# Gumo-A/hnsw_rs

Measured on AMD Instinct MI355X. Metric: queries/sec at recall@10>=0.99, 1M x 100d L2, higher is better.
Workload: dtype f32

## Files before the change

### hnsw_rs_amd/csrc/search_lean.hip

```cpp

#include <algorithm>
#include <cstdlib>

#include "device_index.h"
#include "launch.h"
#include "search_common.h"
#include "switches.h"

namespace hx {
namespace {

#define HX_LIKELY(x) __builtin_expect(!!(x), 1)
#define HX_UNLIKELY(x) __builtin_expect(!!(x), 0)

constexpr u64 LK_INVALID = ~0ull;
constexpr u64 LK_MASK = 0x7FFFFFFFFFFFFFFFull;
constexpr u64 LK_EXPANDED = 1ull << 63;

struct LeanArgs {
    const float *rows;
    const uint32_t *adj0;
    const uint32_t *adj_up;
    const uint32_t *upper_base;
    const uint32_t *ovf_off, *ovf_nbrs;
    const float *Q;
    const uint32_t *qsel;
    uint32_t *out_ids;
    float *out_dists;
    uint32_t *out_counts;
    hnsw_query_stats *out_stats;
    uint32_t n_points, ep, nb_layers, S0, S1, ef, n, slots_log2;
    unsigned long long *dbg;
    uint32_t *spill_tab;
    uint32_t spill_log2;
    uint32_t lds_limit;
};

#ifdef HX_STAMPS
__device__ __forceinline__ unsigned long long stamp_now() {
    __builtin_amdgcn_sched_barrier(0);
    asm volatile("s_waitcnt vmcnt(0) lgkmcnt(0)" ::: "memory");
    const unsigned long long t = __builtin_readcyclecounter();
    asm volatile("s_waitcnt lgkmcnt(0)" ::: "memory");
    __builtin_amdgcn_sched_barrier(0);
    return t;
}
#define STAMP(var) const unsigned long long var = stamp_now()
#define STAMP_ADD(slot, a, b) dbg_acc[slot] += (b) - (a)
#else
#define STAMP(var)
#define STAMP_ADD(slot, a, b)
#endif

__device__ __forceinline__ uint32_t rdlane(uint32_t v, uint32_t l) {
    return (uint32_t)__builtin_amdgcn_readlane((int)v, (int)l);
}
__device__ __forceinline__ u64 rdlane64(u64 v, uint32_t l) {
    return ((u64)rdlane((uint32_t)(v >> 32), l) << 32) | rdlane((uint32_t)v, l);
}
__device__ __forceinline__ uint32_t uni(uint32_t x) { return (uint32_t)__builtin_amdgcn_readfirstlane((int)x); }
__device__ __forceinline__ void lds_fence() { asm volatile("s_waitcnt lgkmcnt(0)" ::: "memory"); }
template <int CTRL>
__device__ __forceinline__ uint32_t dpp_or_max(uint32_t x) {
    return (uint32_t)__builtin_amdgcn_update_dpp(-1, (int)x, CTRL, 0xF, 0xF, false);
}
__device__ __forceinline__ uint32_t wave_min_u32(uint32_t v) {
    v = min(v, dpp_or_max<0xB1>(v));
    v = min(v, dpp_or_max<0x4E>(v));
    v = min(v, dpp_or_max<0x141>(v));
    v = min(v, dpp_or_max<0x140>(v));
    return min(min(rdlane(v, 0), rdlane(v, 16)), min(rdlane(v, 32), rdlane(v, 48)));
}

struct Visited {
    uint32_t *tab;
    uint32_t bshift, bmask;

    __device__ __forceinline__ uint32_t home(uint32_t id) const { return (id * 0x9E3779B1u) >> bshift; }

    __device__ __forceinline__ uint32_t look(uint32_t id, uint32_t b) const {
        const uint4 bk = *reinterpret_cast<const uint4 *>(tab + 4 * b);
        const uint32_t m = min(min(bk.x ^ id, bk.y ^ id), min(bk.z ^ id, bk.w ^ id));
        const uint32_t nf = 4u + (uint32_t)(((int32_t)bk.x >> 31) + ((int32_t)bk.y >> 31) + ((int32_t)bk.z >> 31) +
                                            ((int32_t)bk.w >> 31));
        return m == 0 ? 4u : (nf == 4u ? 5u : nf);
    }
    __device__ __forceinline__ uint32_t claim(uint32_t id, uint32_t b, uint32_t t) const {
        uint32_t old = 0;
        if (t < 4u) old = atomicCAS(tab + 4 * b + t, HX_EMPTY_SLOT, id);
        return old;
    }
    __device__ __forceinline__ bool finish(uint32_t id, uint32_t b, uint32_t t, bool pend, bool fresh) const {
        while (__ballot(pend)) {
            if (pend) {
                if (t == 5u) b = (b + 1) & bmask;
                t = look(id, b);
                const uint32_t old = claim(id, b, t);
                const bool won = old == HX_EMPTY_SLOT;
                fresh |= won;
                pend = (t != 4u) & !won;
            }
        }
        return fresh;
    }
    __device__ __forceinline__ bool insert(uint32_t id, bool ins) const {
        const uint32_t b = home(id);
        uint32_t t = look(id, b);
        t = ins ? t : 4u;
        const uint32_t old = claim(id, b, t);
        const bool fresh = old == HX_EMPTY_SLOT;
        return finish(id, b, t, (t != 4u) & !fresh, fresh);
    }
    __device__ __forceinline__ void clear(uint32_t nslots, int lane) const {
        for (uint32_t s = lane; s < (nslots >> 2); s += 64)
            reinterpret_cast<uint4 *>(tab)[s] = make_uint4(HX_EMPTY_SLOT, HX_EMPTY_SLOT, HX_EMPTY_SLOT, HX_EMPTY_SLOT);
        lds_fence();
    }

    uint32_t *gtab = nullptr;
    uint32_t gshift = 0, gmask = 0;
    bool spill = false;

    __device__ __forceinline__ bool g_contains(uint32_t id) const {
        uint32_t s = ((id * 0x9E3779B1u) >> gshift) & gmask;
        while (true) {
            const uint32_t cur = __hip_atomic_load(gtab + s, __ATOMIC_RELAXED, __HIP_MEMORY_SCOPE_AGENT);
            if (cur == id) return true;
            if (cur == HX_EMPTY_SLOT) return false;
            s = (s + 1) & gmask;
        }
    }
    __device__ __forceinline__ uint32_t g_claim(uint32_t id) const {
        uint32_t s = ((id * 0x9E3779B1u) >> gshift) & gmask;
        while (true) {
            const uint32_t old = atomicCAS(gtab + s, HX_EMPTY_SLOT, id);
            if (old == HX_EMPTY_SLOT) return HX_EMPTY_SLOT;
            if (old == id) return id;
            s = (s + 1) & gmask;
        }
    }
    __device__ __forceinline__ void open_second_level(int lane) {
        const uint32_t nslots = gmask + 1;
        for (uint32_t s = lane; s < (nslots >> 2); s += 64)
            reinterpret_cast<uint4 *>(gtab)[s] = make_uint4(HX_EMPTY_SLOT, HX_EMPTY_SLOT, HX_EMPTY_SLOT, HX_EMPTY_SLOT);
        __builtin_amdgcn_fence(__ATOMIC_RELEASE, "agent");
        asm volatile("s_waitcnt vmcnt(0)" ::: "memory");
        spill = true;
    }
    __device__ __forceinline__ uint32_t look2(uint32_t id, uint32_t b, bool probe, bool claim_now) const {
        uint32_t t = look(id, b);
        if (!spill) return t;
        if (!probe) return 4u;
        while (t == 5u) {
            b = (b + 1) & bmask;
            t = look(id, b);
        }
        if (t == 4u) return 4u;
        if (claim_now) return g_claim(id) == HX_EMPTY_SLOT ? 7u : 4u;
        return g_contains(id) ? 4u : 6u;
    }
    __device__ __forceinline__ uint32_t claim2(uint32_t id, uint32_t b, uint32_t t) const {
        uint32_t old = 0;
        if (t < 4u)
            old = atomicCAS(tab + 4 * b + t, HX_EMPTY_SLOT, id);
        else if (t == 6u)
            old = g_claim(id);
        else if (t == 7u)
            old = HX_EMPTY_SLOT;
        return old;
    }
    __device__ __forceinline__ bool finish2(uint32_t id, uint32_t b, uint32_t t, bool pend, bool fresh) const {
        while (__ballot(pend)) {
            if (pend) {
                if (t == 5u) b = (b + 1) & bmask;
                t = look2(id, b, true, false);
                const uint32_t old = claim2(id, b, t);
                const bool won = old == HX_EMPTY_SLOT;
                fresh |= won;
                pend = (t != 4u) & !won;
            }
        }
        return fresh;
    }
};

#ifndef HX_MERGE_SHIFT_MAX
#define HX_MERGE_SHIFT_MAX 2
#endif
template <int R>
struct Lst {
    static constexpr int NR = R;
    struct Masks {
        u64 U[R];
    };
    u64 L[R];
    uint32_t n_cur;
    u64 last_key;

    static __device__ __forceinline__ uint32_t idx_of(int r, int lane) { return (uint32_t)(R * lane + r); }
    __device__ __forceinline__ void set_first(u64 key, int lane) {
        if (lane == 0) L[0] = key;
        n_cur = 1;
    }

    __device__ __forceinline__ void init() {
#pragma unroll
        for (int r = 0; r < R; r++) L[r] = LK_INVALID;
        n_cur = 0;
        last_key = LK_INVALID;
    }
    __device__ __forceinline__ int first_unexp() const {
        uint32_t pos = 0xFFFFFFFFu;
#pragma unroll
        for (int r = 0; r < R; r++) {
            const u64 U = __ballot((int32_t)(uint32_t)(L[r] >> 32) >= 0);
            const uint32_t i = U ? (uint32_t)(R * (__ffsll((long long)U) - 1) + r) : 0xFFFFFFFFu;
            pos = min(pos, i);
        }
        return (int)pos;
    }
    __device__ __forceinline__ void unexp_masks(Masks &mk) const {
#pragma unroll
        for (int r = 0; r < R; r++) mk.U[r] = __ballot((int32_t)(uint32_t)(L[r] >> 32) >= 0);
    }
    __device__ __forceinline__ int take_first(Masks &mk) const {
        u64(&U)[R] = mk.U;
        uint32_t pos = 0xFFFFFFFFu;
#pragma unroll
        for (int r = 0; r < R; r++) {
            const uint32_t i = U[r] ? (uint32_t)(R * (__ffsll((long long)U[r]) - 1) + r) : 0xFFFFFFFFu;
            pos = min(pos, i);
        }
#pragma unroll
        for (int r = 0; r < R; r++)
            if (pos != 0xFFFFFFFFu && (pos % R) == (uint32_t)r) U[r] &= U[r] - 1;
        return (int)pos;
    }
    __device__ __forceinline__ uint32_t id_at(uint32_t pos) const {
        uint32_t v = 0;
#pragma unroll
        for (int r = 0; r < R; r++) {
            const uint32_t t = rdlane((uint32_t)L[r], pos / R);
            if ((pos % R) == (uint32_t)r) v = t;
        }
        return v;
    }
    __device__ __forceinline__ u64 key_at(uint32_t pos) const {
        u64 v = 0;
#pragma unroll
        for (int r = 0; r < R; r++) {
            const u64 t = rdlane64(L[r], pos / R);
            if ((pos % R) == (uint32_t)r) v = t;
        }
        return v;
    }
    __device__ __forceinline__ void mark(uint32_t pos, int lane) {
#pragma unroll
        for (int r = 0; r < R; r++)
            if ((pos % R) == (uint32_t)r && (uint32_t)lane == pos / R) L[r] |= LK_EXPANDED;
    }
    __device__ __forceinline__ void refresh_last(uint32_t ef) {
        last_key = n_cur >= ef ? (key_at(ef - 1) & LK_MASK) : LK_INVALID;
    }

    __device__ __forceinline__ void merge(u64 key, uint32_t ef, u64 *perm, int lane) {
        const bool surv = key < last_key;
        const u64 smask = __ballot(surv);
        if (smask == 0) return;
        const uint32_t m = (uint32_t)__popcll(smask);
        if (m <= HX_MERGE_SHIFT_MAX) {
            u64 it = smask;
            while (it) {
                const uint32_t j = (uint32_t)__ffsll((long long)it) - 1;
                it &= it - 1;
                const u64 e = rdlane64(key, j);
                if (!(e < last_key)) continue;
                uint32_t pos = 0;
#pragma unroll
                for (int r = 0; r < R; r++) pos += (uint32_t)__popcll(__ballot((L[r] & LK_MASK) < e));
                const uint32_t plo = (uint32_t)__builtin_amdgcn_update_dpp(0, (int)(uint32_t)L[R - 1], 0x138, 0xF, 0xF, false);
                const uint32_t phi = (uint32_t)__builtin_amdgcn_update_dpp(0, (int)(uint32_t)(L[R - 1] >> 32), 0x138, 0xF, 0xF, false);
                u64 below = ((u64)phi << 32) | plo;
#pragma unroll
                for (int r = R - 1; r >= 0; r--) {
                    const uint32_t idx = (uint32_t)(R * lane + r);
                    const u64 from = r > 0 ? L[r > 0 ? r - 1 : 0] : below;
                    L[r] = idx < pos ? L[r] : (idx == pos ? e : from);
                }
                n_cur = min(n_cur + 1, ef);
                if (ef < 64u * R) {
#pragma unroll
                    for (int r = 0; r < R; r++)
                        if ((uint32_t)(R * lane + r) >= ef) L[r] = LK_INVALID;
                }
                refresh_last(ef);
            }
            return;
        }
        u64 *sv = perm + 64 * R;
        u64 Lm[R];
        uint32_t shift[R];
#pragma unroll
        for (int r = 0; r < R; r++) {
            Lm[r] = L[r] & LK_MASK;
            shift[r] = 0;
        }
        uint32_t srank = 0;
        u64 it = smask;
        while (it) {
            const uint32_t j = (uint32_t)__ffsll((long long)it) - 1;
            it &= it - 1;
            const u64 e = rdlane64(key, j);
#pragma unroll
            for (int r = 0; r < R; r++) shift[r] += e < Lm[r] ? 1u : 0u;
            srank += e < key ? 1u : 0u;
        }
        const uint32_t n_new = min(n_cur + m, ef);
#pragma unroll
        for (int r = 0; r < R; r++) perm[R * lane + r] = LK_INVALID;
        asm volatile("" ::: "memory");
#pragma unroll
        for (int r = 0; r < R; r++) {
            const uint32_t idx = (uint32_t)(R * lane + r);
            const uint32_t np = idx + shift[r];
            if (idx < n_cur && np < n_new) perm[np] = L[r];
        }
        if (surv) sv[srank] = key;
        asm volatile("" ::: "memory");
        u64 v[R], H[R];
        bool hole[R];
#pragma unroll
        for (int r = 0; r < R; r++) v[r] = perm[R * lane + r];
#pragma unroll
        for (int r = 0; r < R; r++) {
            hole[r] = v[r] == LK_INVALID && (uint32_t)(R * lane + r) < n_new;
            H[r] = __ballot(hole[r]);
        }
#pragma unroll
        for (int r = 0; r < R; r++) {
            uint32_t hr = 0;
#pragma unroll
            for (int r2 = 0; r2 < R; r2++) {
                hr += __builtin_amdgcn_mbcnt_hi((uint32_t)(H[r2] >> 32), __builtin_amdgcn_mbcnt_lo((uint32_t)H[r2], 0u));
                if (r2 < r && hole[r2]) hr++;
            }
            if (hole[r]) v[r] = sv[hr];
        }
#pragma unroll
        for (int r = 0; r < R; r++) L[r] = v[r];
        n_cur = n_new;
        lds_fence();
        refresh_last(ef);
    }
};

struct LstHT {
    static constexpr int NR = 2;
    struct Masks {
        u64 head, tail;
        bool tail_known;
    };
    u64 L[2];
    uint32_t n_cur;
    u64 last_key;

    static __device__ __forceinline__ uint32_t idx_of(int r, int lane) { return (uint32_t)(64 * r + lane); }
    __device__ __forceinline__ void init() {
        L[0] = L[1] = LK_INVALID;
        n_cur = 0;
        last_key = LK_INVALID;
    }
    __device__ __forceinline__ void set_first(u64 key, int lane) {
        if (lane == 0) L[0] = key;
        n_cur = 1;
    }
    __device__ __forceinline__ void unexp_masks(Masks &mk) const {
        mk.head = __ballot((int32_t)(uint32_t)(L[0] >> 32) >= 0);
        mk.tail = 0;
        mk.tail_known = false;
    }
    __device__ __forceinline__ int take_first(Masks &mk) const {
        if (HX_LIKELY(mk.head != 0)) {
            const int pos = __ffsll((long long)mk.head) - 1;
            mk.head &= mk.head - 1;
            return pos;
        }
        if (!mk.tail_known) {
            mk.tail = n_cur > 64 ? __ballot((int32_t)(uint32_t)(L[1] >> 32) >= 0) : 0ull;
            mk.tail_known = true;
        }
        if (mk.tail == 0) return -1;
        const int pos = __ffsll((long long)mk.tail) - 1;
        mk.tail &= mk.tail - 1;
        return 64 + pos;
    }
    __device__ __forceinline__ uint32_t id_at(uint32_t pos) const {
        const uint32_t a = rdlane((uint32_t)L[0], pos & 63u), b = rdlane((uint32_t)L[1], pos & 63u);
        return pos < 64u ? a : b;
    }
    __device__ __forceinline__ u64 key_at(uint32_t pos) const {
        const u64 a = rdlane64(L[0], pos & 63u), b = rdlane64(L[1], pos & 63u);
        return pos < 64u ? a : b;
    }
    __device__ __forceinline__ void mark(uint32_t pos, int lane) {
        if ((uint32_t)lane == pos) L[0] |= LK_EXPANDED;
        if ((uint32_t)lane + 64u == pos) L[1] |= LK_EXPANDED;
    }
    __device__ __forceinline__ void refresh_last(uint32_t ef) {
        last_key = n_cur >= ef ? (rdlane64(L[1], (ef - 65u) & 63u) & LK_MASK) : LK_INVALID;
    }
    static __device__ __forceinline__ u64 shr1(u64 v) {
        const uint32_t lo = (uint32_t)__builtin_amdgcn_update_dpp(0, (int)(uint32_t)v, 0x138, 0xF, 0xF, false);
        const uint32_t hi = (uint32_t)__builtin_amdgcn_update_dpp(0, (int)(uint32_t)(v >> 32), 0x138, 0xF, 0xF, false);
        return ((u64)hi << 32) | lo;
    }

    __device__ __forceinline__ void merge(u64 key, uint32_t ef, u64 *perm, int lane) {
        const bool surv = key < last_key;
        const u64 smask = __ballot(surv);
        if (smask == 0) return;
        const uint32_t m = (uint32_t)__popcll(smask);
        if (m <= HX_MERGE_SHIFT_MAX) {
            u64 it = smask;
            while (it) {
                const uint32_t j = (uint32_t)__ffsll((long long)it) - 1;
                it &= it - 1;
                const u64 e = rdlane64(key, j);
                if (!(e < last_key)) continue;
                const uint32_t pos = (uint32_t)__popcll(__ballot((L[0] & LK_MASK) < e));
                if (pos < 64u) {
                    const u64 carry = rdlane64(L[0], 63);
                    const u64 below = shr1(L[0]);
                    L[0] = (uint32_t)lane < pos ? L[0] : ((uint32_t)lane == pos ? e : below);
                    const u64 tb = shr1(L[1]);
                    L[1] = lane == 0 ? carry : tb;
                } else {
                    const uint32_t tpos = (uint32_t)__popcll(__ballot((L[1] & LK_MASK) < e));
                    const u64 tb = shr1(L[1]);
                    L[1] = (uint32_t)lane < tpos ? L[1] : ((uint32_t)lane == tpos ? e : tb);
                }
                n_cur = min(n_cur + 1, ef);
                if (64u + (uint32_t)lane >= ef) L[1] = LK_INVALID;
                refresh_last(ef);
            }
            return;
        }
        u64 *sv = perm + 128;
        const u64 Mm = L[0] & LK_MASK, Tm = L[1] & LK_MASK;
        uint32_t sh0 = 0, sh1 = 0, srank = 0;
        u64 it = smask;
        while (it) {
            const uint32_t j = (uint32_t)__ffsll((long long)it) - 1;
            it &= it - 1;
            const u64 e = rdlane64(key, j);
            sh0 += e < Mm ? 1u : 0u;
            sh1 += e < Tm ? 1u : 0u;
            srank += e < key ? 1u : 0u;
        }
        const uint32_t n_new = min(n_cur + m, ef);
        perm[lane] = LK_INVALID;
        perm[64 + lane] = LK_INVALID;
        asm volatile("" ::: "memory");
        {
            const uint32_t i0 = (uint32_t)lane, i1 = 64u + (uint32_t)lane;
            if (i0 < n_cur && i0 + sh0 < n_new) perm[i0 + sh0] = L[0];
            if (i1 < n_cur && i1 + sh1 < n_new) perm[i1 + sh1] = L[1];
        }
        if (surv) sv[srank] = key;
        asm volatile("" ::: "memory");
        u64 v0 = perm[lane], v1 = perm[64 + lane];
        const bool hole0 = v0 == LK_INVALID && (uint32_t)lane < n_new;
        const bool hole1 = v1 == LK_INVALID && 64u + (uint32_t)lane < n_new;
        const u64 H0 = __ballot(hole0), H1 = __ballot(hole1);
        const uint32_t hr0 = __builtin_amdgcn_mbcnt_hi((uint32_t)(H0 >> 32), __builtin_amdgcn_mbcnt_lo((uint32_t)H0, 0u));
        const uint32_t hr1 = (uint32_t)__popcll(H0) +
                             __builtin_amdgcn_mbcnt_hi((uint32_t)(H1 >> 32), __builtin_amdgcn_mbcnt_lo((uint32_t)H1, 0u));
        if (hole0) v0 = sv[hr0];
        if (hole1) v1 = sv[hr1];
        L[0] = v0;
        L[1] = v1;
        n_cur = n_new;
        lds_fence();
        refresh_last(ef);
    }
};

template <int DS>
__device__ __forceinline__ float chain_sum(const uint4 (&w)[DS / 4], const float (&qv)[DS]) {
    float s = 0.0f;
#pragma unroll
    for (int p = 0; p < DS / 4; p++) {
        const uint32_t dw[4] = {w[p].x, w[p].y, w[p].z, w[p].w};
#pragma unroll
        for (int j = 0; j < 4; j += 2) {
            const f32x2 x = {__builtin_bit_cast(float, dw[j]), __builtin_bit_cast(float, dw[j + 1])};
            const f32x2 y = {qv[4 * p + j], qv[4 * p + j + 1]};
            const f32x2 t = x - y;
            const f32x2 t2 = t * t;
            s += t2.x;
            s += t2.y;
        }
    }
    return s;
}
template <int DS>
__device__ __forceinline__ float row_dist(const float *rows, uint32_t id, bool want, const float (&qv)[DS]) {
    float s = 0.0f;
    if (want) {
        const uint4 *src = reinterpret_cast<const uint4 *>(rows + (size_t)id * DS);
        uint4 w[DS / 4];
#pragma unroll
        for (int p = 0; p < DS / 4; p++) w[p] = src[p];
        __builtin_amdgcn_sched_barrier(0);
        s = chain_sum<DS>(w, qv);
    }
    return __builtin_sqrtf(s);
}

template <int DS, class LT, int CK = 4>
__global__ void __launch_bounds__(64) hx_lean_f32_kernel(const LeanArgs a) {
    constexpr int R = LT::NR;
    static_assert(DS % 4 == 0, "whole 16-byte pieces");
    constexpr bool COOP = coop_rows<HNSW_VEC_F32, DS>();
    constexpr bool SPILLV = R >= 6;
    extern __shared__ __attribute__((aligned(16))) unsigned char smem[];
    const int lane = threadIdx.x;
    const uint32_t q = a.qsel ? a.qsel[blockIdx.x] : blockIdx.x;
    const uint32_t hslots = 1u << a.slots_log2;
    u64 *perm = reinterpret_cast<u64 *>(smem + 4ull * hslots);
    unsigned char *coop_img = reinterpret_cast<unsigned char *>(perm);
    uint32_t *coop_ids = reinterpret_cast<uint32_t *>(coop_img + HX_COOP_IMG_BYTES);
    Visited vis;
    vis.tab = reinterpret_cast<uint32_t *>(smem);

    uint32_t n_dist = 0, n_exp = 0, sum_deg = 0, n_vis = 0;
    int32_t status = HNSW_OK;
#ifdef HX_STAMPS
    unsigned long long dbg_acc[16] = {0, 0, 0, 0, 0, 0, 0, 0, 0, 0, 0, 0, 0, 0, 0, 0};
    const unsigned long long t_begin = __builtin_readcyclecounter();
#endif

    const float *qp = a.Q + (size_t)q * DS;
    QueryRegs<DS> qreg;
    float(&qv)[DS] = qreg.v;
#pragma unroll
    for (int e = 0; e < DS; e++) qv[e] = qp[e];
    {
        bool bad = false;
        for (int e = lane; e < DS; e += 64) {
            const float x = qp[e];
            bad |= (x != x);
        }
        if (__ballot(bad)) status = HNSW_ERR_NAN_INPUT;
    }
#pragma unroll
    for (int e = 0; e < DS; e++) asm volatile("" : "+v"(qv[e]));

    auto dist_of = [&](uint32_t id, bool want) __attribute__((always_inline)) -> float {
        if constexpr (COOP) {
            return __builtin_sqrtf(f32_rows_coop<DS, CK, true, true>(reinterpret_cast<const uint8_t *>(a.rows), id, want, qreg,
                                                                    coop_ids, coop_img, lane));
        } else {
            return row_dist<DS>(a.rows, id, want, qv);
        }
    };

    u64 best = LK_INVALID;
    uint32_t cur = a.ep;
    if (status == HNSW_OK) {
        if (cur >= a.n_points) {
            status = HNSW_ERR_ARG;
        } else {
            const float d0 = dist_of(cur, lane == 0);
            const uint32_t bits = rdlane(__builtin_bit_cast(uint32_t, d0), 0);
            n_dist = 1;
            if (__builtin_bit_cast(float, bits) != __builtin_bit_cast(float, bits))
                status = HNSW_ERR_NAN_INPUT;
            else
                best = ((u64)bits << 32) | cur;
        }
    }

    const uint32_t up_slots = max(hslots >> 2, 64u);
    uint32_t ub_cur = HX_EMPTY_SLOT;
    bool have_ub = false;
    for (int layer = (int)a.nb_layers - 1; layer >= 1 && status == HNSW_OK; layer--) {
        vis.bshift = 32 - (__ffs((int)up_slots) - 1 - 2);
        vis.bmask = (up_slots >> 2) - 1;
        const uint32_t vis_limit = up_slots - (up_slots >> 2);
        vis.clear(up_slots, lane);
        vis.insert(cur, lane == 0);
        n_vis = 1;
        if (!have_ub) {
            ub_cur = uni(a.upper_base[cur]);
            have_ub = true;
        }
        while (status == HNSW_OK) {
            if (ub_cur == HX_EMPTY_SLOT) {
                status = HNSW_ERR_NODE_NOT_IN_GRAPH;
                break;
            }
            n_exp++;
            bool improved = false;
            uint32_t new_cur = cur, new_ub = ub_cur;
            const uint32_t *row = a.adj_up + ((size_t)ub_cur + (uint32_t)layer - 1) * a.S1;
            uint32_t ovf_lo = 0, ovf_hi = 0;
            bool first = true;
            while (true) {
                uint32_t nb = HX_EMPTY_SLOT;
                if (first) {
                    if ((uint32_t)lane < a.S1) nb = row[lane];
                } else {
                    if (ovf_lo + lane < ovf_hi) nb = a.ovf_nbrs[ovf_lo + lane];
                    ovf_lo += 64;
                }
                const bool valid = (int32_t)nb >= 0;
                if (first) {
                    const u64 pm = __ballot((int32_t)nb < 0 && nb != HX_EMPTY_SLOT);
                    if (HX_UNLIKELY(pm != 0)) {
                        const uint32_t o = rdlane(nb, (uint32_t)__ffsll((long long)pm) - 1) & ~HX_OVF_FLAG;
                        ovf_lo = uni(a.ovf_off[o]);
                        ovf_hi = uni(a.ovf_off[o + 1]);
                    }
                    first = false;
                }
                const uint32_t cnt = (uint32_t)__popcll(__ballot(valid));
                sum_deg += cnt;
                if (HX_LIKELY(cnt != 0)) {
                    if (HX_UNLIKELY(n_vis + cnt > vis_limit)) {
                        status = HNSW_ERR_OVERFLOW;
                        break;
                    }
                    const bool fresh = vis.insert(nb, valid);
                    const u64 fm = __ballot(fresh);
                    const uint32_t nf = (uint32_t)__popcll(fm);
                    n_vis += nf;
                    n_dist += nf;
                    if (HX_LIKELY(fm != 0)) {
                        uint32_t ubn = HX_EMPTY_SLOT;
                        if (fresh) ubn = a.upper_base[nb];
                        const float dist = dist_of(nb, fresh);
                        const bool nan = fresh && dist != dist;
                        if (HX_UNLIKELY(__ballot(nan) != 0)) {
                            status = HNSW_ERR_NAN_INPUT;
                            break;
                        }
                        const uint32_t db = fresh ? __builtin_bit_cast(uint32_t, dist) : 0xFFFFFFFFu;
                        const uint32_t mn = wave_min_u32(db);
                        u64 tie = __ballot(fresh && db == mn);
                        uint32_t j = (uint32_t)__ffsll((long long)tie) - 1;
                        uint32_t bid = rdlane(nb, j);
                        tie &= tie - 1;
                        while (tie) {
                            const uint32_t j2 = (uint32_t)__ffsll((long long)tie) - 1;
                            tie &= tie - 1;
                            const uint32_t id2 = rdlane(nb, j2);
                            if (id2 < bid) {
                                bid = id2;
                                j = j2;
                            }
                        }
                        const u64 k = ((u64)mn << 32) | bid;
                        if (k < best) {
                            best = k;
                            new_cur = bid;
                            new_ub = rdlane(ubn, j);
                            improved = true;
                        }
                    }
                }
                if (HX_LIKELY(ovf_lo >= ovf_hi)) break;
            }
            if (!improved || status != HNSW_OK) break;
            cur = new_cur;
            ub_cur = new_ub;
        }
    }

#ifdef HX_STAMPS
    dbg_acc[7] = __builtin_readcyclecounter() - t_begin;
#endif
    const uint32_t ef = max(1u, a.ef);
    LT lst;
    lst.init();
    if (status == HNSW_OK) {
        vis.bshift = 32 - (a.slots_log2 - 2);
        vis.bmask = (hslots >> 2) - 1;
        uint32_t lds_limit = hslots - (hslots >> 2);
        if constexpr (SPILLV) {
            if (a.spill_tab != nullptr && a.lds_limit != 0) lds_limit = min(lds_limit, max(128u, a.lds_limit));
        }
        uint32_t vis_limit = lds_limit;
        if constexpr (SPILLV) {
            if (a.spill_tab != nullptr) {
                vis.gtab = a.spill_tab + ((size_t)blockIdx.x << a.spill_log2);
                vis.gmask = (1u << a.spill_log2) - 1;
                vis.gshift = 32 - a.spill_log2;
                vis_limit = lds_limit + (1u << a.spill_log2) / 2;
            }
        }
        vis.clear(hslots, lane);
        vis.insert(cur, lane == 0);
        n_vis = 1;
        lst.set_first(best, lane);
        lst.refresh_last(ef);
        const uint32_t S0 = a.S0;
        const bool upper = lane >= 32;
        const uint32_t slot = (uint32_t)lane & 31u;
        uint32_t pre_nb = HX_EMPTY_SLOT, pre_c = HX_EMPTY_SLOT, pre_p = HX_EMPTY_SLOT;

        uint32_t ovf_lo = 0, ovf_hi = 0;

        while (true) {
            STAMP(f0);
            if constexpr (SPILLV) {
                if (HX_UNLIKELY(!vis.spill && vis.gtab != nullptr && n_vis + 64u > lds_limit)) vis.open_second_level(lane);
            }
            int ppos = -1;
            uint32_t pid = HX_EMPTY_SLOT;
            uint32_t nb = HX_EMPTY_SLOT;
            const bool ovf_pass = ovf_lo < ovf_hi;
            if (HX_UNLIKELY(ovf_pass)) {
                if (lane < 32 && ovf_lo + (uint32_t)lane < ovf_hi) nb = a.ovf_nbrs[ovf_lo + (uint32_t)lane];
                ovf_lo += 32;
            } else {
                typename LT::Masks U;
                lst.unexp_masks(U);
                const int cpos = lst.take_first(U);
                if (HX_UNLIKELY(cpos < 0)) break;
                ppos = lst.take_first(U);
                const uint32_t cid = lst.id_at((uint32_t)cpos);
                if (ppos >= 0) pid = lst.id_at((uint32_t)ppos);
                lst.mark((uint32_t)cpos, lane);
                n_exp++;
                if (HX_LIKELY(pre_c == cid && pre_p == pid)) {
                    nb = pre_nb;
                } else {
                    if (slot < S0 && (!upper || ppos >= 0)) nb = a.adj0[(size_t)(upper ? pid : cid) * S0 + slot];
                }
                pre_c = HX_EMPTY_SLOT;
            }
#ifdef HX_STAMPS
            asm volatile("s_waitcnt vmcnt(0)" ::: "memory");
            dbg_acc[6]++;
#endif
            STAMP(f1);
            STAMP_ADD(0, f0, f1);
            const u64 pm = ovf_pass ? 0ull : __ballot((int32_t)nb < -1);
            const bool spec_ok = ppos >= 0 && (pm >> 32) == 0;
            const bool valid = (int32_t)nb >= 0 && (!upper || spec_ok);
            const uint32_t vb = vis.home(nb);
            uint32_t vt0;
            if constexpr (SPILLV)
                vt0 = vis.look2(nb, vb, valid, valid && !upper);
            else
                vt0 = vis.look(nb, vb);
            const uint32_t vt = valid ? vt0 : 4u;
            const bool want_pre = vt != 4u;
            const uint32_t ct = upper ? 4u : vt;
            bool fresh = false;
            float dist = 0.0f;
            if constexpr (COOP) {
                const uint32_t old = SPILLV ? vis.claim2(nb, vb, ct) : vis.claim(nb, vb, ct);
                fresh = old == HX_EMPTY_SLOT;
                const bool pend = (ct != 4u) & !fresh;
                if (HX_UNLIKELY(__ballot(pend) != 0)) fresh = SPILLV ? vis.finish2(nb, vb, ct, pend, fresh) : vis.finish(nb, vb, ct, pend, fresh);
                dist = dist_of(nb, upper ? want_pre : fresh);
            } else if (want_pre) {
                const uint4 *src = reinterpret_cast<const uint4 *>(a.rows + (size_t)nb * DS);
                uint4 w[DS / 4];
#pragma unroll
                for (int p = 0; p < DS / 4; p++) w[p] = src[p];
                __builtin_amdgcn_sched_barrier(0);
                const uint32_t old = SPILLV ? vis.claim2(nb, vb, ct) : vis.claim(nb, vb, ct);
                fresh = old == HX_EMPTY_SLOT;
                const bool pend = (ct != 4u) & !fresh;
                if (HX_UNLIKELY(__ballot(pend) != 0)) {
                    fresh = SPILLV ? vis.finish2(nb, vb, ct, pend, fresh) : vis.finish(nb, vb, ct, pend, fresh);
#ifdef HX_STAMPS
                    dbg_acc[11]++;
#endif
                }
                __builtin_amdgcn_sched_barrier(0);
#ifdef HX_STAMPS
                __builtin_amdgcn_sched_barrier(0);
                asm volatile("s_waitcnt lgkmcnt(0)" ::: "memory");
                const unsigned long long g0 = __builtin_readcyclecounter();
                asm volatile("s_waitcnt lgkmcnt(0)" ::: "memory");
                const unsigned long long g1 = stamp_now();
                dbg_acc[2] += g1 - g0;
#endif
                const float s = chain_sum<DS>(w, qv);
                dist = __builtin_sqrtf(s);
#ifdef HX_STAMPS
                asm volatile("" ::"v"(dist) : "memory");
                dbg_acc[3] += stamp_now() - g1;
#endif
            }
            const bool want = upper ? want_pre : fresh;
            const u64 vmask = __ballot(valid), fmask = __ballot(fresh);
            const uint32_t cnt_c = (uint32_t)__popcll(vmask & 0xFFFFFFFFull);
            const uint32_t cnt_p = (uint32_t)__popcll(vmask >> 32);
            const uint32_t nf_c = (uint32_t)__popcll(fmask);
            sum_deg += cnt_c;
            n_vis += nf_c;
            n_dist += nf_c;
            if (HX_UNLIKELY(n_vis > vis_limit)) {
                status = HNSW_ERR_OVERFLOW;
                break;
            }
            const bool nan = want && dist != dist;
            u64 key = LK_INVALID;
            if (want && !nan) key = ((u64)__builtin_bit_cast(uint32_t, dist) << 32) | nb;
            STAMP(f2);
            STAMP_ADD(1, f1, f2);
            STAMP(f3);
#ifdef HX_STAMPS
            {
                const uint32_t mm = (uint32_t)__popcll(__ballot(!upper && key < lst.last_key));
                if (mm == 0) dbg_acc[12]++; else if (mm <= 2) dbg_acc[13]++; else dbg_acc[14]++;
            }
#endif
            const u64 nanm = __ballot(nan);
            if (HX_UNLIKELY((nanm & 0xFFFFFFFFull) != 0)) {
                status = HNSW_ERR_NAN_INPUT;
                break;
            }
            lst.merge(upper ? LK_INVALID : key, ef, perm, lane);
            STAMP(f3b);
            STAMP_ADD(8, f3, f3b);
            if (HX_UNLIKELY((pm & 0xFFFFFFFFull) != 0)) {
                const uint32_t c_ovf = rdlane(nb, (uint32_t)__ffsll((long long)(pm & 0xFFFFFFFFull)) - 1) & ~HX_OVF_FLAG;
                ovf_lo = uni(a.ovf_off[c_ovf]);
                ovf_hi = uni(a.ovf_off[c_ovf + 1]);
                if (ovf_lo < ovf_hi) continue;
            }
            if (HX_UNLIKELY(!spec_ok)) continue;
            typename LT::Masks V;
            lst.unexp_masks(V);
            const int npos = lst.take_first(V);
            if (HX_UNLIKELY(npos < 0)) break;
            if (HX_UNLIKELY(lst.id_at((uint32_t)npos) != pid)) continue;
            {
                const int apos = lst.take_first(V);
                if (HX_LIKELY(apos >= 0)) {
                    const int bpos = lst.take_first(V);
                    pre_c = lst.id_at((uint32_t)apos);
                    pre_p = bpos >= 0 ? lst.id_at((uint32_t)bpos) : HX_EMPTY_SLOT;
                    pre_nb = HX_EMPTY_SLOT;
                    if (slot < S0 && (!upper || bpos >= 0)) pre_nb = a.adj0[(size_t)(upper ? pre_p : pre_c) * S0 + slot];
                }
            }
            STAMP(f4);
            STAMP_ADD(9, f3b, f4);
            lst.mark((uint32_t)npos, lane);
            n_exp++;
            const uint32_t pt = upper ? vt : 4u;
            const uint32_t pold = SPILLV ? vis.claim2(nb, vb, pt) : vis.claim(nb, vb, pt);
            bool pfresh = pold == HX_EMPTY_SLOT;
            const bool ppend = (pt == 5u) | ((pt < 4u) & !pfresh & (pold != nb));
            if (HX_UNLIKELY(__ballot(ppend) != 0))
                pfresh = SPILLV ? vis.finish2(nb, vb, pt == 5u ? 5u : 0u, ppend, pfresh) : vis.finish(nb, vb, pt == 5u ? 5u : 0u, ppend, pfresh);
            const uint32_t nf_p = (uint32_t)__popcll(__ballot(pfresh));
            sum_deg += cnt_p;
            n_vis += nf_p;
            n_dist += nf_p;
            if (HX_UNLIKELY(n_vis > vis_limit)) {
                status = HNSW_ERR_OVERFLOW;
                break;
            }
            if (HX_UNLIKELY(__ballot(pfresh && nan) != 0)) {
                status = HNSW_ERR_NAN_INPUT;
                break;
            }
            STAMP(f4b);
            STAMP_ADD(5, f4, f4b);
#ifdef HX_STAMPS
            {
                const uint32_t mm = (uint32_t)__popcll(__ballot(pfresh && key < lst.last_key));
                if (mm == 0) dbg_acc[12]++; else if (mm <= 2) dbg_acc[13]++; else dbg_acc[14]++;
                dbg_acc[15]++;
            }
#endif
            lst.merge(pfresh ? key : LK_INVALID, ef, perm, lane);
            STAMP(f5);
            STAMP_ADD(10, f4b, f5);
        }
    }

    const uint32_t count = status == HNSW_OK ? min(a.n, lst.n_cur) : 0;
#pragma unroll
    for (int r = 0; r < R; r++) {
        const uint32_t idx = LT::idx_of(r, lane);
        if (idx < a.n) {
            const bool have = idx < count;
            a.out_ids[(size_t)q * a.n + idx] = have ? (uint32_t)lst.L[r] : HX_EMPTY_SLOT;
            if (a.out_dists)
                a.out_dists[(size_t)q * a.n + idx] =
                    have ? __builtin_bit_cast(float, (uint32_t)((lst.L[r] & LK_MASK) >> 32)) : __builtin_inff();
        }
    }
    for (uint32_t idx = 64u * R + lane; idx < a.n; idx += 64) {
        a.out_ids[(size_t)q * a.n + idx] = HX_EMPTY_SLOT;
        if (a.out_dists) a.out_dists[(size_t)q * a.n + idx] = __builtin_inff();
    }
#ifdef HX_STAMPS
    if (lane == 0 && a.dbg) {
        dbg_acc[4] = __builtin_readcyclecounter() - t_begin;
        for (int i = 0; i < 16; i++) a.dbg[(size_t)q * 16 + i] = dbg_acc[i];
    }
#endif
    if (lane == 0) {
        if (a.out_counts) a.out_counts[q] = count;
        hnsw_query_stats st;
        st.n_dist = n_dist;
        st.n_exp = n_exp;
        st.sum_deg = sum_deg;
        st.status = status;
        a.out_stats[q] = st;
    }
}

template <class LT>
__global__ void __launch_bounds__(64) hx_lean_q8_kernel(const LeanArgs a) {
    constexpr int R = LT::NR;
    constexpr bool SPILLV = R >= 6;
    constexpr int DS = 100, P = 4, NQ = 4 * (DS / 8) + DS % 8;
    constexpr uint32_t HALF = 64, ROW = 128, NCH4 = 4 * (DS / 8), REM = DS % 8;
    extern __shared__ __attribute__((aligned(16))) unsigned char smem[];
    const int lane = threadIdx.x;
    const int h = lane & 1;
    const uint32_t cslot = (uint32_t)lane >> 1;
    const uint32_t q = a.qsel ? a.qsel[blockIdx.x] : blockIdx.x;
    const uint32_t hslots = 1u << a.slots_log2;
    u64 *perm = reinterpret_cast<u64 *>(smem + 4ull * hslots);
    float *yq = reinterpret_cast<float *>(perm + 64 * R + 64);
    Visited vis;
    vis.tab = reinterpret_cast<uint32_t *>(smem);
    const uint8_t *rows8 = reinterpret_cast<const uint8_t *>(a.rows);

    uint32_t n_dist = 0, n_exp = 0, sum_deg = 0, n_vis = 0;
    int32_t status = HNSW_OK;
#ifdef HX_STAMPS
    unsigned long long dbg_acc[16] = {0, 0, 0, 0, 0, 0, 0, 0, 0, 0, 0, 0, 0, 0, 0, 0};
    const unsigned long long t_begin = __builtin_readcyclecounter();
#endif

    QRegs<NQ> qreg;
    {
        DevView dv{};
        dv.dim = DS;
        dv.half_bytes = HALF;
        dv.nch4 = NCH4;
        dv.rem = REM;
        if (!stage_query<HNSW_VEC_QUANT8>(dv, a.Q + (size_t)q * DS, yq, lane)) status = HNSW_ERR_NAN_INPUT;
#pragma unroll
        for (int e = 0; e < NQ; e++) qreg.v[e] = yq[h * (HALF - 8) + e];
    }
    auto eval = [&](uint32_t id, bool want) __attribute__((always_inline)) -> float {
        float acc[4] = {0.0f, 0.0f, 0.0f, 0.0f};
        if (want) {
            const uint4 *src = reinterpret_cast<const uint4 *>(rows8 + (size_t)id * ROW + (size_t)h * HALF);
            uint4 w[P];
#pragma unroll
            for (int p = 0; p < P; p++) w[p] = src[p];
            __builtin_amdgcn_sched_barrier(0);
            quant_half_sums<P, DS>(w, qreg, h, NCH4, REM, acc);
        }
        const float b0 = pair_swap(acc[0]), b1 = pair_swap(acc[1]), b2 = pair_swap(acc[2]), b3 = pair_swap(acc[3]);
        float s = 0.0f;
        s += acc[0];
        s += acc[1];
        s += acc[2];
        s += acc[3];
        s += b0;
        s += b1;
        s += b2;
        s += b3;
        return __builtin_sqrtf(s);
    };
    auto pair_insert = [&](uint32_t id, bool ins) __attribute__((always_inline)) -> bool {
        bool f;
        if constexpr (SPILLV) {
            const bool mine = ins && h == 0;
            const uint32_t b0 = vis.home(id);
            const uint32_t t0 = vis.look2(id, b0, mine, mine);
            const uint32_t t = mine ? t0 : 4u;
            const uint32_t old = vis.claim2(id, b0, t);
            f = old == HX_EMPTY_SLOT;
            f = vis.finish2(id, b0, t, (t != 4u) & !f, f);
        } else {
            f = vis.insert(id, ins && h == 0);
        }
        return (pair_swap_i(f ? 1 : 0) | (f ? 1 : 0)) != 0;
    };

    u64 best = LK_INVALID;
    uint32_t cur = a.ep;
    if (status == HNSW_OK) {
        if (cur >= a.n_points) {
            status = HNSW_ERR_ARG;
        } else {
            const float d0 = eval(cur, lane < 2);
            const uint32_t bits = rdlane(__builtin_bit_cast(uint32_t, d0), 0);
            n_dist = 1;
            if (__builtin_bit_cast(float, bits) != __builtin_bit_cast(float, bits))
                status = HNSW_ERR_NAN_INPUT;
            else
                best = ((u64)bits << 32) | cur;
        }
    }

    const uint32_t up_slots = max(hslots >> 2, 64u);
    uint32_t ub_cur = HX_EMPTY_SLOT;
    bool have_ub = false;
    for (int layer = (int)a.nb_layers - 1; layer >= 1 && status == HNSW_OK; layer--) {
        vis.bshift = 32 - (__ffs((int)up_slots) - 1 - 2);
        vis.bmask = (up_slots >> 2) - 1;
        const uint32_t vis_limit = up_slots - (up_slots >> 2);
        vis.clear(up_slots, lane);
        vis.insert(cur, lane == 0);
        n_vis = 1;
        if (!have_ub) {
            ub_cur = uni(a.upper_base[cur]);
            have_ub = true;
        }
        while (status == HNSW_OK) {
            if (ub_cur == HX_EMPTY_SLOT) {
                status = HNSW_ERR_NODE_NOT_IN_GRAPH;
                break;
            }
            n_exp++;
            bool improved = false;
            uint32_t new_cur = cur, new_ub = ub_cur;
            const uint32_t *row = a.adj_up + ((size_t)ub_cur + (uint32_t)layer - 1) * a.S1;
            uint32_t ovf_lo = 0, ovf_hi = 0;
            for (uint32_t c0 = 0; c0 < a.S1 || ovf_lo < ovf_hi; c0 += 32) {
                uint32_t nb = HX_EMPTY_SLOT;
                if (c0 < a.S1) {
                    if (c0 + cslot < a.S1) nb = row[c0 + cslot];
                    const u64 pm = __ballot((int32_t)nb < -1);
                    if (HX_UNLIKELY(pm != 0)) {
                        const uint32_t o = rdlane(nb, (uint32_t)__ffsll((long long)pm) - 1) & ~HX_OVF_FLAG;
                        ovf_lo = uni(a.ovf_off[o]);
                        ovf_hi = uni(a.ovf_off[o + 1]);
                    }
                } else {
                    if (ovf_lo + cslot < ovf_hi) nb = a.ovf_nbrs[ovf_lo + cslot];
                    ovf_lo += 32;
                }
                const bool valid = (int32_t)nb >= 0;
                const uint32_t cnt = (uint32_t)__popcll(__ballot(valid && h == 0));
                sum_deg += cnt;
                if (cnt == 0) continue;
                if (n_vis + cnt > vis_limit) {
                    status = HNSW_ERR_OVERFLOW;
                    break;
                }
                const bool fresh = pair_insert(nb, valid);
                const u64 fm = __ballot(fresh && h == 0);
                const uint32_t nf = (uint32_t)__popcll(fm);
                n_vis += nf;
                n_dist += nf;
                if (fm == 0) continue;
                uint32_t ubn = HX_EMPTY_SLOT;
                if (fresh && h == 0) ubn = a.upper_base[nb];
                const float dist = eval(nb, fresh);
                const bool mine = fresh && h == 0;
                if (__ballot(mine && dist != dist)) {
                    status = HNSW_ERR_NAN_INPUT;
                    break;
                }
                const uint32_t db = mine ? __builtin_bit_cast(uint32_t, dist) : 0xFFFFFFFFu;
                const uint32_t mn = wave_min_u32(db);
                u64 tie = __ballot(mine && db == mn);
                uint32_t j = (uint32_t)__ffsll((long long)tie) - 1;
                uint32_t bid = rdlane(nb, j);
                tie &= tie - 1;
                while (tie) {
                    const uint32_t j2 = (uint32_t)__ffsll((long long)tie) - 1;
                    tie &= tie - 1;
                    const uint32_t id2 = rdlane(nb, j2);
                    if (id2 < bid) {
                        bid = id2;
                        j = j2;
                    }
                }
                const u64 k = ((u64)mn << 32) | bid;
                if (k < best) {
                    best = k;
                    new_cur = bid;
                    new_ub = rdlane(ubn, j);
                    improved = true;
                }
            }
            if (!improved || status != HNSW_OK) break;
            cur = new_cur;
            ub_cur = new_ub;
        }
    }

#ifdef HX_STAMPS
    dbg_acc[7] = __builtin_readcyclecounter() - t_begin;
#endif
    const uint32_t ef = max(1u, a.ef);
    LT lst;
    lst.init();
    if (status == HNSW_OK) {
        vis.bshift = 32 - (a.slots_log2 - 2);
        vis.bmask = (hslots >> 2) - 1;
        uint32_t lds_limit = hslots - (hslots >> 2);
        if constexpr (SPILLV) {
            if (a.spill_tab != nullptr && a.lds_limit != 0) lds_limit = min(lds_limit, max(128u, a.lds_limit));
        }
        uint32_t vis_limit = lds_limit;
        if constexpr (SPILLV) {
            if (a.spill_tab != nullptr) {
                vis.gtab = a.spill_tab + ((size_t)blockIdx.x << a.spill_log2);
                vis.gmask = (1u << a.spill_log2) - 1;
                vis.gshift = 32 - a.spill_log2;
                vis_limit = lds_limit + (1u << a.spill_log2) / 2;
            }
        }
        vis.clear(hslots, lane);
        vis.insert(cur, lane == 0);
        n_vis = 1;
        lst.set_first(best, lane);
        lst.refresh_last(ef);
        const uint32_t S0 = a.S0;
        uint32_t pre_nb = HX_EMPTY_SLOT, pre_c = HX_EMPTY_SLOT;

        while (true) {
            STAMP(f0);
            if constexpr (SPILLV) {
                if (HX_UNLIKELY(!vis.spill && vis.gtab != nullptr && n_vis + 64u > lds_limit)) vis.open_second_level(lane);
            }
            typename LT::Masks U;
            lst.unexp_masks(U);
            const int cpos = lst.take_first(U);
            if (cpos < 0) break;
            const int ppos = lst.take_first(U);
            const uint32_t cid = lst.id_at((uint32_t)cpos);
            lst.mark((uint32_t)cpos, lane);
            n_exp++;
            uint32_t nb;
            if (pre_c == cid) {
                nb = pre_nb;
            } else {
                nb = HX_EMPTY_SLOT;
                if (cslot < S0) nb = a.adj0[(size_t)cid * S0 + cslot];
            }
            pre_c = HX_EMPTY_SLOT;
            if (ppos >= 0) {
                pre_c = lst.id_at((uint32_t)ppos);
                pre_nb = HX_EMPTY_SLOT;
                if (cslot < S0) pre_nb = a.adj0[(size_t)pre_c * S0 + cslot];
            }
            const u64 pm = __ballot((int32_t)nb < -1);
#ifdef HX_STAMPS
            dbg_acc[6]++;
#endif
            STAMP(f1);
            STAMP_ADD(0, f0, f1);
            const bool valid = (int32_t)nb >= 0;
            const uint32_t vb = vis.home(nb);
            uint32_t vt0;
            if constexpr (SPILLV)
                vt0 = vis.look2(nb, vb, valid && h == 0, valid && h == 0);
            else
                vt0 = vis.look(nb, vb);
            const uint32_t ct = (valid && h == 0) ? vt0 : 4u;
            const uint32_t old = SPILLV ? vis.claim2(nb, vb, ct) : vis.claim(nb, vb, ct);
            bool fresh0 = old == HX_EMPTY_SLOT;
            const bool pend = (ct != 4u) & !fresh0;
            if (__ballot(pend)) fresh0 = SPILLV ? vis.finish2(nb, vb, ct, pend, fresh0) : vis.finish(nb, vb, ct, pend, fresh0);
            const bool fresh = (pair_swap_i(fresh0 ? 1 : 0) | (fresh0 ? 1 : 0)) != 0;
            const u64 vmask = __ballot(valid && h == 0), fmask = __ballot(fresh0);
            const uint32_t nf = (uint32_t)__popcll(fmask);
            sum_deg += (uint32_t)__popcll(vmask);
            n_vis += nf;
            n_dist += nf;
            if (HX_UNLIKELY(n_vis > vis_limit)) {
                status = HNSW_ERR_OVERFLOW;
                break;
            }
            STAMP(f2);
            STAMP_ADD(1, f1, f2);
            u64 key = LK_INVALID;
            if (fmask) {
                const float dist = eval(nb, fresh);
                const bool mine = fresh0;
                if (__ballot(mine && dist != dist)) {
                    status = HNSW_ERR_NAN_INPUT;
                    break;
                }
                if (mine) key = ((u64)__builtin_bit_cast(uint32_t, dist) << 32) | nb;
            }
            STAMP(f3);
            STAMP_ADD(3, f2, f3);
            lst.merge(key, ef, perm, lane);
            STAMP(f4);
            STAMP_ADD(8, f3, f4);
            if (pm) {
                const uint32_t c_ovf = rdlane(nb, (uint32_t)__ffsll((long long)pm) - 1) & ~HX_OVF_FLAG;
                const uint32_t lo = uni(a.ovf_off[c_ovf]), hi = uni(a.ovf_off[c_ovf + 1]);
                for (uint32_t base = lo; base < hi && status == HNSW_OK; base += 32) {
                    const uint32_t i = base + cslot;
                    const bool ov = i < hi;
                    const uint32_t onb = ov ? a.ovf_nbrs[i] : HX_EMPTY_SLOT;
                    const uint32_t ocnt = (uint32_t)__popcll(__ballot(ov && h == 0));
                    sum_deg += ocnt;
                    if (n_vis + ocnt > vis_limit) {
                        status = HNSW_ERR_OVERFLOW;
                        break;
                    }
                    if constexpr (SPILLV) {
                        if (HX_UNLIKELY(!vis.spill && vis.gtab != nullptr && n_vis + 64u > lds_limit)) vis.open_second_level(lane);
                    }
                    const bool ofresh = pair_insert(onb, ov);
                    const uint32_t onf = (uint32_t)__popcll(__ballot(ofresh && h == 0));
                    n_vis += onf;
                    n_dist += onf;
                    if (onf == 0) continue;
                    const float odist = eval(onb, ofresh);
                    const bool omine = ofresh && h == 0;
                    if (__ballot(omine && odist != odist)) {
                        status = HNSW_ERR_NAN_INPUT;
                        break;
                    }
                    lst.merge(omine ? (((u64)__builtin_bit_cast(uint32_t, odist) << 32) | onb) : LK_INVALID, ef, perm,
                              lane);
                }
                if (status != HNSW_OK) break;
            }
        }
    }

    const uint32_t count = status == HNSW_OK ? min(a.n, lst.n_cur) : 0;
#pragma unroll
    for (int r = 0; r < R; r++) {
        const uint32_t idx = LT::idx_of(r, lane);
        if (idx < a.n) {
            const bool have = idx < count;
            a.out_ids[(size_t)q * a.n + idx] = have ? (uint32_t)lst.L[r] : HX_EMPTY_SLOT;
            if (a.out_dists)
                a.out_dists[(size_t)q * a.n + idx] =
                    have ? __builtin_bit_cast(float, (uint32_t)((lst.L[r] & LK_MASK) >> 32)) : __builtin_inff();
        }
    }
    for (uint32_t idx = 64u * R + lane; idx < a.n; idx += 64) {
        a.out_ids[(size_t)q * a.n + idx] = HX_EMPTY_SLOT;
        if (a.out_dists) a.out_dists[(size_t)q * a.n + idx] = __builtin_inff();
    }
#ifdef HX_STAMPS
    if (lane == 0 && a.dbg) {
        dbg_acc[4] = __builtin_readcyclecounter() - t_begin;
        for (int i = 0; i < 16; i++) a.dbg[(size_t)q * 16 + i] = dbg_acc[i];
    }
#endif
    if (lane == 0) {
        if (a.out_counts) a.out_counts[q] = count;
        hnsw_query_stats st;
        st.n_dist = n_dist;
        st.n_exp = n_exp;
        st.sum_deg = sum_deg;
        st.status = status;
        a.out_stats[q] = st;
    }
}

#include "pair_kernel.inc"

template <class LT>
int launch_lean_q8(const LeanArgs &a_in, uint32_t nblocks, hipStream_t stream) {
    constexpr int R = LT::NR;
    LeanArgs a = a_in;
    VisitedSpill sp(R >= 6 && a.slots_log2 >= 13, a, a.slots_log2, nblocks, stream);
    const size_t lds = (4ull << a.slots_log2) + (64ull * R + 64) * 8 + 2 * 56 * 4;
    return launch_checked({"search kernel launch", "search needs %zu bytes of LDS (> 160 KiB)"}, hx_lean_q8_kernel<LT>,
                          dim3(nblocks), dim3(64), lds, stream, a);
}

template <int DS, class LT, int CK = 4>
int launch_lean_one(const LeanArgs &a_in, uint32_t nblocks, hipStream_t stream) {
    constexpr int R = LT::NR;
    LeanArgs a = a_in;
    VisitedSpill sp(R >= 6 && a.slots_log2 >= 13, a, a.slots_log2, nblocks, stream);
    const size_t lds = (4ull << a.slots_log2) +
                       std::max<size_t>((64ull * R + 64) * 8, coop_rows<HNSW_VEC_F32, DS>() ? HX_COOP_IMG_BYTES + 256 : 0);
    return launch_checked({"search kernel launch", "search needs %zu bytes of LDS (> 160 KiB)"}, hx_lean_f32_kernel<DS, LT, CK>,
                          dim3(nblocks), dim3(64), lds, stream, a);
}

}

bool lean_applicable(const DevView &v, const SearchArgs &a, uint32_t ef_max) {
    if (!sw::lean()) return false;
    const bool f32_ok = v.kind == HNSW_VEC_F32 && ((v.dim == 100 && v.row_stride == 400) ||
                                                     (sw::lean_128() && v.dim == 128 && v.row_stride == 512));
    const bool q8_ok = sw::lean_q8_enabled() && v.kind == HNSW_VEC_QUANT8 && v.dim == 100 && v.row_stride == 128 && v.half_bytes == 64;
    if (!f32_ok && !q8_ok) return false;
    if (a.entries != nullptr || a.layer_lo != 0 || a.layer_hi != (int32_t)v.nb_layers - 1) return false;
    if (a.layer_hi > 0 && a.ef_upper != 1) return false;
    const bool to512 = (v.dim == 100 && (v.kind == HNSW_VEC_F32 || sw::lean_q8_wide())) || (v.dim == 128 && v.kind == HNSW_VEC_F32);
    if (v.S0 > 32 || v.S1 > 64 || ef_max > (sw::lean_wide() ? (to512 ? 512u : 256u) : 128u) || (a.flags & 1u)) return false;
    return true;
}

int launch_lean(const DevView &v, const SearchArgs &s, uint32_t nblocks, uint32_t slots_log2, hipStream_t stream) {
    LeanArgs a{};
    a.rows = reinterpret_cast<const float *>(v.rows);
    a.adj0 = v.adj0;
    a.adj_up = v.adj_up;
    a.upper_base = v.upper_base;
    a.ovf_off = v.ovf_off;
    a.ovf_nbrs = v.ovf_nbrs;
    a.Q = s.Q;
    a.qsel = s.qsel;
    a.out_ids = s.out_ids;
    a.out_dists = s.out_dists;
    a.out_counts = s.out_counts;
    a.out_stats = s.out_stats;
    a.n_points = v.n_points;
    a.ep = v.ep;
    a.nb_layers = v.nb_layers;
    a.S0 = v.S0;
    a.S1 = v.S1;
    a.ef = s.ef_bottom;
    a.n = s.n;
    a.slots_log2 = slots_log2;
    a.dbg = s.dbg;
    if (v.kind == HNSW_VEC_QUANT8) {
        if (a.ef <= 64) return launch_lean_q8<Lst<1>>(a, nblocks, stream);
        if (a.ef > 448) return launch_lean_q8<Lst<8>>(a, nblocks, stream);
        if (a.ef > 384) return launch_lean_q8<Lst<7>>(a, nblocks, stream);
        if (a.ef > 320) return launch_lean_q8<Lst<6>>(a, nblocks, stream);
        if (a.ef > 256) return launch_lean_q8<Lst<5>>(a, nblocks, stream);
        if (a.ef > 128) return launch_lean_q8<Lst<4>>(a, nblocks, stream);
        return launch_lean_q8<LstHT>(a, nblocks, stream);
    }
    if (v.dim == 128) {
        const bool few = nblocks <= 4 * cu_count();
        if (a.ef <= 64) return few ? launch_lean_one<128, Lst<1>, 4>(a, nblocks, stream) : launch_lean_one<128, Lst<1>, 2>(a, nblocks, stream);
        if (a.ef > 384) return launch_lean_one<128, Lst<8>, 2>(a, nblocks, stream);
        if (a.ef > 256) return launch_lean_one<128, Lst<6>, 2>(a, nblocks, stream);
        if (a.ef > 128) return launch_lean_one<128, Lst<4>, 2>(a, nblocks, stream);
        return few ? launch_lean_one<128, LstHT, 4>(a, nblocks, stream) : launch_lean_one<128, LstHT, 2>(a, nblocks, stream);
    }
    if (sw::pair_mode() != 0 && a.ef <= 128 && a.qsel == nullptr) {
        if (a.ef <= 64) return launch_pair<100, Lst<1>>(a, nblocks, stream);
        return launch_pair<100, LstHT>(a, nblocks, stream);
    }
    if (a.ef <= 64) return launch_lean_one<100, Lst<1>>(a, nblocks, stream);
    if (a.ef > 448) return launch_lean_one<100, Lst<8>>(a, nblocks, stream);
    if (a.ef > 384) return launch_lean_one<100, Lst<7>>(a, nblocks, stream);
    if (a.ef > 320) return launch_lean_one<100, Lst<6>>(a, nblocks, stream);
    if (a.ef > 256) return launch_lean_one<100, Lst<5>>(a, nblocks, stream);
    if (a.ef > 128) return launch_lean_one<100, Lst<4>>(a, nblocks, stream);
    return launch_lean_one<100, LstHT>(a, nblocks, stream);
}

}
```

Measured before the change: 6.035 million.

## Prefetch adjacency for predicted next candidates when new neighbors beat speculative pair

When freshly computed neighbor keys fall below the speculatively paired candidate's key, the kernel predicts the next two expansion candidates from the best new keys. It then issues their adjacency loads early so the next iteration can reuse them. For small list sizes it also carries over the already computed distance when the upper half's pair is unchanged, skipping a row reload. This adds a serial readlane scan and extra loads on mispredictions, and debug stamp slots grow to 26.

```diff
diff --git a/hnsw_rs_amd/csrc/search_lean.hip b/hnsw_rs_amd/csrc/search_lean.hip
--- a/hnsw_rs_amd/csrc/search_lean.hip
+++ b/hnsw_rs_amd/csrc/search_lean.hip
@@ -47,6 +47,7 @@
 }
 #define STAMP(var) const unsigned long long var = stamp_now()
 #define STAMP_ADD(slot, a, b) dbg_acc[slot] += (b) - (a)
+constexpr int HX_LEAN_DBG_SLOTS = 26;
 #else
 #define STAMP(var)
 #define STAMP_ADD(slot, a, b)
@@ -523,6 +524,8 @@
     static_assert(DS % 4 == 0, "whole 16-byte pieces");
     constexpr bool COOP = coop_rows<HNSW_VEC_F32, DS>();
     constexpr bool SPILLV = R >= 6;
+    constexpr bool MISS_AHEAD = !COOP && !SPILLV;
+    constexpr bool MISS_KEEP = MISS_AHEAD && R <= 2;
     extern __shared__ __attribute__((aligned(16))) unsigned char smem[];
     const int lane = threadIdx.x;
     const uint32_t q = a.qsel ? a.qsel[blockIdx.x] : blockIdx.x;
@@ -536,8 +539,10 @@
     uint32_t n_dist = 0, n_exp = 0, sum_deg = 0, n_vis = 0;
     int32_t status = HNSW_OK;
 #ifdef HX_STAMPS
-    unsigned long long dbg_acc[16] = {0, 0, 0, 0, 0, 0, 0, 0, 0, 0, 0, 0, 0, 0, 0, 0};
+    unsigned long long dbg_acc[HX_LEAN_DBG_SLOTS] = {0, 0, 0, 0, 0, 0, 0, 0, 0, 0, 0, 0, 0, 0, 0, 0, 0, 0, 0, 0, 0, 0, 0, 0, 0, 0};
     const unsigned long long t_begin = __builtin_readcyclecounter();
+    bool dbg_follow = false, dbg_took_pre = false;
+    uint32_t dbg_pred_c = HX_EMPTY_SLOT, dbg_pred_p = HX_EMPTY_SLOT, dbg_old_p = HX_EMPTY_SLOT;
 #endif
 
     const float *qp = a.Q + (size_t)q * DS;
@@ -708,6 +713,8 @@
         const bool upper = lane >= 32;
         const uint32_t slot = (uint32_t)lane & 31u;
         uint32_t pre_nb = HX_EMPTY_SLOT, pre_c = HX_EMPTY_SLOT, pre_p = HX_EMPTY_SLOT;
+        bool carry = false;
+        float kdist = 0.0f;
 
         uint32_t ovf_lo = 0, ovf_hi = 0;
 
@@ -718,6 +725,8 @@
             }
             int ppos = -1;
             uint32_t pid = HX_EMPTY_SLOT;
+            u64 pkey = 0;
+            bool kept = false;
             uint32_t nb = HX_EMPTY_SLOT;
             const bool ovf_pass = ovf_lo < ovf_hi;
             if (HX_UNLIKELY(ovf_pass)) {
@@ -730,15 +739,32 @@
                 if (HX_UNLIKELY(cpos < 0)) break;
                 ppos = lst.take_first(U);
                 const uint32_t cid = lst.id_at((uint32_t)cpos);
-                if (ppos >= 0) pid = lst.id_at((uint32_t)ppos);
+                if constexpr (MISS_AHEAD) {
+                    if (ppos >= 0) {
+                        pkey = lst.key_at((uint32_t)ppos);
+                        pid = (uint32_t)pkey;
+                    }
+                } else {
+                    if (ppos >= 0) pid = lst.id_at((uint32_t)ppos);
+                }
                 lst.mark((uint32_t)cpos, lane);
                 n_exp++;
+#ifdef HX_STAMPS
+                if (dbg_follow) {
+                    if (cid == dbg_pred_c && pid == dbg_pred_p) dbg_acc[19]++;
+                    if (pid == dbg_old_p) dbg_acc[20]++;
+                    dbg_follow = false;
+                }
+                dbg_took_pre = pre_c == cid && pre_p == pid;
+#endif
                 if (HX_LIKELY(pre_c == cid && pre_p == pid)) {
                     nb = pre_nb;
+                    if constexpr (MISS_KEEP) kept = carry;
                 } else {
                     if (slot < S0 && (!upper || ppos >= 0)) nb = a.adj0[(size_t)(upper ? pid : cid) * S0 + slot];
                 }
                 pre_c = HX_EMPTY_SLOT;
+                carry = false;
             }
 #ifdef HX_STAMPS
             asm volatile("s_waitcnt vmcnt(0)" ::: "memory");
@@ -746,6 +772,12 @@
 #endif
             STAMP(f1);
             STAMP_ADD(0, f0, f1);
+#ifdef HX_STAMPS
+            if (!ovf_pass && dbg_took_pre) {
+                dbg_acc[21] += f1 - f0;
+                dbg_acc[22]++;
+            }
+#endif
             const u64 pm = ovf_pass ? 0ull : __ballot((int32_t)nb < -1);
             const bool spec_ok = ppos >= 0 && (pm >> 32) == 0;
             const bool valid = (int32_t)nb >= 0 && (!upper || spec_ok);
@@ -759,14 +791,15 @@
             const bool want_pre = vt != 4u;
             const uint32_t ct = upper ? 4u : vt;
             bool fresh = false;
-            float dist = 0.0f;
+            const bool keptl = MISS_KEEP && kept && upper;
+            float dist = keptl ? kdist : 0.0f;
             if constexpr (COOP) {
                 const uint32_t old = SPILLV ? vis.claim2(nb, vb, ct) : vis.claim(nb, vb, ct);
                 fresh = old == HX_EMPTY_SLOT;
                 const bool pend = (ct != 4u) & !fresh;
                 if (HX_UNLIKELY(__ballot(pend) != 0)) fresh = SPILLV ? vis.finish2(nb, vb, ct, pend, fresh) : vis.finish(nb, vb, ct, pend, fresh);
                 dist = dist_of(nb, upper ? want_pre : fresh);
-            } else if (want_pre) {
+            } else if (want_pre && !keptl) {
                 const uint4 *src = reinterpret_cast<const uint4 *>(a.rows + (size_t)nb * DS);
                 uint4 w[DS / 4];
 #pragma unroll
@@ -814,6 +847,12 @@
             if (want && !nan) key = ((u64)__builtin_bit_cast(uint32_t, dist) << 32) | nb;
             STAMP(f2);
             STAMP_ADD(1, f1, f2);
+#ifdef HX_STAMPS
+            if (kept) {
+                dbg_acc[23] += f2 - f1;
+                dbg_acc[24]++;
+            }
+#endif
             STAMP(f3);
 #ifdef HX_STAMPS
             {
@@ -825,6 +864,45 @@
             if (HX_UNLIKELY((nanm & 0xFFFFFFFFull) != 0)) {
                 status = HNSW_ERR_NAN_INPUT;
                 break;
+            }
+            if constexpr (MISS_AHEAD) {
+                const u64 bm = __ballot(!upper && key < pkey);
+                if (HX_UNLIKELY(bm != 0) && spec_ok && pm == 0) {
+                    u64 k1 = rdlane64(key, (uint32_t)__ffsll((long long)bm) - 1), k2 = LK_INVALID;
+                    u64 rest = bm & (bm - 1);
+                    if (rest != 0) {
+                        const u64 t2 = rdlane64(key, (uint32_t)__ffsll((long long)rest) - 1);
+                        rest &= rest - 1;
+                        k2 = max(k1, t2);
+                        k1 = min(k1, t2);
+                        for (int i = 2; i < 32 && rest != 0; i++) {
+                            const u64 t = rdlane64(key, (uint32_t)__ffsll((long long)rest) - 1);
+                            rest &= rest - 1;
+                            k2 = t < k1 ? k1 : min(k2, t);
+                            k1 = min(k1, t);
+                        }
+                    }
+                    const bool again = k2 == LK_INVALID;
+#ifdef HX_STAMPS
+                    {
+                        const uint32_t nbel = (uint32_t)__popcll(bm);
+                        if (nbel == 1) dbg_acc[16]++; else if (nbel == 2) dbg_acc[17]++; else dbg_acc[18]++;
+                        dbg_follow = true;
+                        dbg_pred_c = (uint32_t)k1;
+                        dbg_pred_p = again ? pid : (uint32_t)k2;
+                        dbg_old_p = pid;
+                    }
+#endif
+                    pre_c = (uint32_t)k1;
+                    pre_p = again ? pid : (uint32_t)k2;
+                    const bool held = upper && again;
+                    pre_nb = held ? nb : HX_EMPTY_SLOT;
+                    if (slot < S0 && !held) pre_nb = a.adj0[(size_t)(upper ? pre_p : pre_c) * S0 + slot];
+                    if constexpr (MISS_KEEP) {
+                        carry = again;
+                        kdist = dist;
+                    }
+                }
             }
             lst.merge(upper ? LK_INVALID : key, ef, perm, lane);
             STAMP(f3b);
@@ -907,7 +985,7 @@
 #ifdef HX_STAMPS
     if (lane == 0 && a.dbg) {
         dbg_acc[4] = __builtin_readcyclecounter() - t_begin;
-        for (int i = 0; i < 16; i++) a.dbg[(size_t)q * 16 + i] = dbg_acc[i];
+        for (int i = 0; i < HX_LEAN_DBG_SLOTS; i++) a.dbg[(size_t)q * HX_LEAN_DBG_SLOTS + i] = dbg_acc[i];
     }
 #endif
     if (lane == 0) {
@@ -1255,7 +1333,7 @@
 #ifdef HX_STAMPS
     if (lane == 0 && a.dbg) {
         dbg_acc[4] = __builtin_readcyclecounter() - t_begin;
-        for (int i = 0; i < 16; i++) a.dbg[(size_t)q * 16 + i] = dbg_acc[i];
+        for (int i = 0; i < 16; i++) a.dbg[(size_t)q * HX_LEAN_DBG_SLOTS + i] = dbg_acc[i];
     }
 #endif
     if (lane == 0) {
```

New measurement: 6.177 million (median of 6 runs). +2.4%, better.
